# applied-geodesy/bundle-adjustment

Measured on AMD Instinct MI355X. Metric: LM iterations/sec, higher is better.
Workload: dtype f64

## Files before the change

bundle-adjustment_amd/csrc/cholflow.h:

```cpp
#pragma once
#include <hip/hip_runtime.h>
#include <limits.h>
#include <stddef.h>

#include <vector>

#include "devbuf.h"

namespace jaicov {

enum { FACTOR_DEFAULT = 0, FACTOR_STREAMS = 1, FACTOR_TWO_STEP = 2, FACTOR_ONE_KERNEL = 3, FACTOR_CHAIN2 = 4, FACTOR_CHAIN3 = 5 };

constexpr int HOOK_UNSET = INT_MIN;
struct FlowHooks {
    int form = FACTOR_DEFAULT;
    int min_blocks = HOOK_UNSET;
    int split_m = 0, split_from = 0;
    int timeout_ms = HOOK_UNSET;
    bool trace_on = false;
    int chain8_min_nb = HOOK_UNSET;
    bool chain_trace = false;
    bool verbose = false;
};
FlowHooks flow_hooks();

struct FlowDecision {
    bool use_flow;
    bool one_kernel;
    bool chain;
    int second;
    int split_m, split_from;
};
FlowDecision flow_decide(int nb, bool kernels_overlap, const FlowHooks &h);
int chain8_min_blocks(const FlowHooks &h);

enum { FLOW_TICKET = 0, FLOW_ABORT = 1, FLOW_DIAG_NEXT = 2, FLOW_CHAIN_AT = 3, FLOW_STALE = 4, FLOW_STALE_CONFIRMED = 5, FLOW_RESCUED = 6, FLOW_WG_OFF = 7, FLOW_CTRL_WORDS = 16 };
constexpr int FLOW_MAX_GRID = 1024;

struct FlowLayout {
    size_t done;
    size_t applied;
    size_t diag_ready;
    size_t factored;
    size_t wgstate;
    size_t wgsnap;
    size_t pflag;
    size_t words;
};
FlowLayout flow_layout(int nb, int row_blocks, int partials);

struct FlowView {
    double *L;
    long ld;
    double *invd;
    int *d_info;
    int nfact, n;
    hipStream_t stream;
    hipStream_t pstream;
    hipStream_t dstream;
};

struct FlowCounters { long long stale_events = 0, stale_confirmed = 0, rescued = 0; };

class FlowFactor {
  public:
    hipError_t init(const FlowView &view, const FlowHooks &hooks);
    bool ready() const { return ready_; }
    void set_source(const double *N, long ldN, const double *V, const double *Bh, int bstride, int d, int U) {
        src_ = N; src_ld_ = ldN; V_ = V; Bh_ = Bh; bstride_ = bstride; d_ = d; U_ = U;
    }
    hipError_t factor(hipEvent_t all_ready, bool profile);
    const int *abort_word() const { return ready_ ? flags_.get() + FLOW_ABORT : nullptr; }
    hipError_t read_ctrl(int (&cw)[8]) const;
    bool collect(const int (&cw)[8]);
    void report_stall() const;
    bool elapsed_ms(float *ms);
    hipError_t enable_trace(bool on);
    const long long *trace() const { return trace_.get(); }
    size_t trace_words() const { return ((size_t)n_tasks() + v_.nfact / 128) * 8; }
    int n_tasks() const { return (int)tasks_host_.size(); }
    const FlowCounters &counters() const { return counters_; }

  private:
    FlowView v_{};
    bool ready_ = false, timed_ = false;
    bool one_kernel_ = false, chain_ = false;
    int second_ = 0;
    int grid_ = 0;
    int keep_ = 0;
    int partials_ = 0;
    FlowLayout lay_{};
    int wg_off_ = 0;
    std::vector<int4> tasks_host_;
    DevBuf<int4> tasks_;
    DevBuf<int> flags_;
    DevBuf<double> scratch_;
    DevBuf<double> partial_;
    DevBuf<long long> trace_;
    DevBuf<double> diag_scratch_;
    HostMapped<int> alive_;
    int seq_ = 0;
    DevEvent e0_, e1_, t0_, t1_;
    const double *src_ = nullptr, *V_ = nullptr, *Bh_ = nullptr;
    long src_ld_ = 0;
    int d_ = 0, U_ = 0, bstride_ = 0;
    FlowCounters counters_;
};

}
```

bundle-adjustment_amd/csrc/cholflow.hip:

```cpp
#include <hip/hip_runtime.h>
#include <stdio.h>
#include <stdlib.h>
#include <string.h>

#include <algorithm>
#include <chrono>
#include <mutex>
#include <thread>
#include <vector>

#include "dense.h"
#include "gemm_f64.h"
#include "potrf_diag.h"

namespace jaicov {

#define HIPCHK(x)                                  \
    do {                                           \
        hipError_t _e = (x);                       \
        if (_e != hipSuccess) return _e;           \
    } while (0)

constexpr int FLOW_FIN = 1 << 20;
constexpr int FLOW_PART = 1 << 21;
// ... 3 lines not shown
constexpr int FLOW_STAGE = GEMM_BK * 2 * FLOW_LDS;

struct FlowArgs {
    double *L;
    long ld;
    double *invd;
    const int4 *tasks;
    int n_tasks;
    int nb;
    int fs;
    int *ctrl;
    int *done;
    int *applied;
    int *diag_ready;
    int *factored;
    int *info;
    int *alive;
    int seq;
    const double *src;
    long src_ld;
    const double *V;
    const double *Bh;
    int d, U, bstride;
    double *diag_scratch;
    const double *zeros;
    double *scratch;
    double *partial;
    int *pflag;
    long long timeout;
    int fake_a;
    int crit_prio;
    int keep;
    int second_wg;
    int second_update;
    int inv_wt;
    int crit_span;
    int *wgstate;
    long long *ctrace;
    long long *trace;
};

__device__ __forceinline__ int flow_ld(const int *p) { return __hip_atomic_load(p, __ATOMIC_RELAXED, __HIP_MEMORY_SCOPE_AGENT); }
__device__ __forceinline__ int flow_ld_rmw(const int *p) { return __hip_atomic_fetch_or(const_cast<int *>(p), 0, __ATOMIC_RELAXED, __HIP_MEMORY_SCOPE_AGENT); }
__device__ __forceinline__ void flow_st(int *p, int v) { __hip_atomic_store(p, v, __ATOMIC_RELAXED, __HIP_MEMORY_SCOPE_SYSTEM); }
__device__ __forceinline__ int flow_ld_sys(const int *p) { return __hip_atomic_load(p, __ATOMIC_RELAXED, __HIP_MEMORY_SCOPE_SYSTEM); }
__device__ __forceinline__ void store_wt(double *p, double v) {
// ... 191 lines not shown
                const double *src = phase != 0 || part ? g.zeros + (tq & 15)
                                    : scaled   ? g.src + ((long)ti * 128 + trow) * g.src_ld + (long)tj * 128 + tcol
                                               : g.L + ((long)ti * 128 + trow) * g.ld + (long)tj * 128 + tcol;
                const long sld = phase != 0 || part ? 0 : (scaled ? g.src_ld : g.ld);
#pragma unroll
                for (int x = 0; x < 4; x++)
#pragma unroll
                    for (int r = 0; r < 4; r++) {
                        const double *rowp = src + (long)(16 * x + 4 * r) * sld;
#pragma unroll
                        for (int y = 0; y < 4; y++) acc[x][y][r] = rowp[16 * y];
                    }
                if (scaled) {
                    const int R0 = ti * 128 + (int)trow, C0 = tj * 128 + (int)tcol;
                    double vc[4];
#pragma unroll
                    for (int y = 0; y < 4; y++) vc[y] = g.V[C0 + 16 * y];
#pragma unroll
                    for (int x = 0; x < 4; x++)
#pragma unroll
                        for (int r = 0; r < 4; r++) {
                            const int R = R0 + 16 * x + 4 * r;
                            const double vr = g.V[R];
#pragma unroll
                            for (int y = 0; y < 4; y++) {
                                const int Cc = C0 + 16 * y;
                                double v = vr * acc[x][y][r] * vc[y];
                                for (int a = 0; a < g.d; a++) v += g.Bh[(long)a * g.bstride + R] * g.Bh[(long)a * g.bstride + Cc];
                                const bool inside = R >= g.d && R < g.U && Cc >= g.d;
                                acc[x][y][r] = inside ? v : (R == Cc ? 1.0 : 0.0);
                            }
                        }
                }
            }
            if (g.trace && phase == 0) { t_c = wall_clock64(); c_c = clock64(); }
            for (bool more = true; more;) {
                const double *Ap, *Bp;
                long lda, ldb;
                int nk;
                double asign;
                if (phase == 0) {
                    if (k >= k1) break;
                    FLOW_STAGE_MARK(k, 3);
                    if (tid < 64) {
                        FLOW_OPAQUE_TID(lane);
                        const int *fi = g.done + (long)ti * g.fs, *fj = g.done + (long)tj * g.fs;
                        const long long t0 = wall_clock64();
                        int spins = 0, cnt = 0;
                        for (;;) {
                            const int idx = k + lane;
                            const bool ready = idx < k1 && flow_ld(fi + idx) != 0 && flow_ld(fj + idx) != 0;
                            const unsigned long long m = __ballot(ready);
                            cnt = m == ~0ull ? 64 : __builtin_ctzll(~m);
// ... 483 lines not shown
        if (tr) tr[4] = wall_clock64();
    }
}

FlowHooks flow_hooks() {
    FlowHooks h;
    if (const char *e = getenv("JAICOV_FACTOR_FORM")) {
        if (!strcmp(e, "streams")) h.form = FACTOR_STREAMS;
        else if (!strcmp(e, "two_step")) h.form = FACTOR_TWO_STEP;
        else if (!strcmp(e, "one_kernel")) h.form = FACTOR_ONE_KERNEL;
        else if (!strcmp(e, "chain2")) h.form = FACTOR_CHAIN2;
        else if (!strcmp(e, "chain3")) h.form = FACTOR_CHAIN3;
    }
    if (const char *e = getenv("JAICOV_FLOW_MIN_BLOCKS")) h.min_blocks = atoi(e);
    if (const char *e = getenv("JAICOV_FLOW_SPLIT")) {
        int a = 1, b = 0;
        if (sscanf(e, "%d:%d", &a, &b) >= 1) { h.split_m = a < 1 ? 1 : a; h.split_from = b; }
    }
    if (const char *e = getenv("JAICOV_FLOW_TIMEOUT_MS")) h.timeout_ms = atoi(e);
    h.trace_on = getenv("JAICOV_FLOW_TRACE_ON") != nullptr;
    if (const char *e = getenv("JAICOV_CHAIN8_MIN_NB")) h.chain8_min_nb = atoi(e);
    h.chain_trace = getenv("JAICOV_CHAIN_TRACE") != nullptr;
    h.verbose = getenv("JAICOV_VERBOSE") != nullptr;
    return h;
}

int chain8_min_blocks(const FlowHooks &h) { return h.chain8_min_nb != HOOK_UNSET ? h.chain8_min_nb : 24; }

FlowDecision flow_decide(int nb, bool kernels_overlap, const FlowHooks &h) {
    FlowDecision dec{};
    dec.use_flow = h.form != FACTOR_STREAMS && nb >= (h.min_blocks != HOOK_UNSET ? h.min_blocks : 12);
    if (dec.use_flow) {
        dec.one_kernel = !kernels_overlap || h.form == FACTOR_ONE_KERNEL;
        dec.chain = !dec.one_kernel && h.form != FACTOR_TWO_STEP;
        dec.second = dec.chain && h.form != FACTOR_CHAIN2 && (nb < 80 || h.form == FACTOR_CHAIN3) ? 2 : 0;
    }
    dec.split_m = 1; dec.split_from = 1 << 30;
    if (nb >= 80) { dec.split_m = 2; dec.split_from = nb / 2; }
    if (h.split_m > 0) { dec.split_m = h.split_m; dec.split_from = h.split_from; }
    return dec;
}

FlowLayout flow_layout(int nb, int row_blocks, int partials) {
    FlowLayout l{};
    l.done = FLOW_CTRL_WORDS;
    l.applied = l.done + (size_t)row_blocks * nb;
    l.diag_ready = l.applied + (size_t)row_blocks * nb;
    l.factored = l.diag_ready + nb;
    l.wgstate = l.factored + nb;
    l.wgsnap = l.wgstate + FLOW_MAX_GRID;
    l.pflag = l.wgsnap + FLOW_MAX_GRID;
    l.words = l.pflag + (size_t)partials;
    return l;
}

static std::vector<int4> flow_schedule(int nb, int row_blocks, int w, bool chain, int second, int split_m = 1, int split_from = 1 << 30, int *n_bufs = nullptr) {
    std::vector<int4> tasks;
    tasks.reserve((size_t)nb * (row_blocks + 1) / 2 + row_blocks);
    if (w < 1) w = 1;
    if (split_m > 8) split_m = 8;
    if (w > 1) split_m = 1;
    int bufs = 0;
    auto task = [&](int i, int j) {
// ... 34 lines not shown
    return tasks;
}

}
extern "C" int jaicov_debug_flow_tasks2(int nb, int row_blocks, int w, int chain, int second, int split_m, int split_from, int *out, int cap) {
    if (nb < 1 || row_blocks < nb) return -1;
    const std::vector<int4> t = jaicov::flow_schedule(nb, row_blocks, w, chain != 0, second, split_m, split_from);
    for (size_t q = 0; q < t.size() && (int)q < cap; q++) {
        out[4 * q] = t[q].x; out[4 * q + 1] = t[q].y; out[4 * q + 2] = t[q].z; out[4 * q + 3] = t[q].w;
    }
    return (int)t.size();
}
extern "C" int jaicov_debug_flow_tasks(int nb, int row_blocks, int w, int chain, int second, int *out, int cap) {
    return jaicov_debug_flow_tasks2(nb, row_blocks, w, chain, second, 1, 1 << 30, out, cap);
}
extern "C" void jaicov_debug_flow_split(int nb, int *m, int *from) {
    const jaicov::FlowDecision dec = jaicov::flow_decide(nb, true, jaicov::flow_hooks());
    *m = dec.split_m; *from = dec.split_from;
}
extern "C" void jaicov_debug_flow_decision(int nb, int kernels_overlap, int *out6) {
    const jaicov::FlowDecision dec = jaicov::flow_decide(nb, kernels_overlap != 0, jaicov::flow_hooks());
    out6[0] = dec.use_flow; out6[1] = dec.one_kernel; out6[2] = dec.chain; out6[3] = dec.second; out6[4] = dec.split_m; out6[5] = dec.split_from;
}
extern "C" int jaicov_debug_flow_layout(int nb, int row_blocks, int partials, long long *out8) {
    if (nb < 1 || row_blocks < nb || partials < 0) return -1;
    const jaicov::FlowLayout l = jaicov::flow_layout(nb, row_blocks, partials);
    const size_t w[8] = {l.done, l.applied, l.diag_ready, l.factored, l.wgstate, l.wgsnap, l.pflag, l.words};
    for (int i = 0; i < 8; i++) out8[i] = (long long)w[i];
    return jaicov::FLOW_MAX_GRID;
}
namespace jaicov {

__global__ void flow_probe_wait_kernel(int *word, int *result) {
    const long long t0 = wall_clock64();
    int seen = 0;
    while (wall_clock64() - t0 < 5000000LL) {
        if (__hip_atomic_load(word, __ATOMIC_RELAXED, __HIP_MEMORY_SCOPE_AGENT) != 0) { seen = 1; break; }
        __builtin_amdgcn_s_sleep(20);
    }
    *result = seen;
}
__global__ void flow_probe_set_kernel(int *word) { __hip_atomic_store(word, 1, __ATOMIC_RELAXED, __HIP_MEMORY_SCOPE_AGENT); }

static bool flow_kernels_overlap(hipStream_t dstream) {
    static int cached = -1;
    static std::mutex cache_mutex;
// ... 103 lines not shown
    return std::max(1, std::min(FLOW_MAX_GRID, 2 * (cus > 0 ? cus : 256)));
}
extern "C" int jaicov_debug_flow_residency(int *out8) {
    hipStream_t s = nullptr;
    StreamLease d(STREAM_DIAGONAL_CUS);
    if (!d.get() || hipStreamCreateWithFlags(&s, hipStreamNonBlocking) != hipSuccess) return -1;
    const FlowResidency r = flow_measure_residency(s, d.get(), flow_grid_size(), 2);
    hipStreamDestroy(s);
    out8[0] = r.valid; out8[1] = r.n_xcd; out8[2] = r.n_se; out8[3] = r.dealt; out8[4] = r.resident_min; out8[5] = r.queued_max; out8[6] = r.keep; out8[7] = r.se_cap;
    return 0;
}

hipError_t FlowFactor::init(const FlowView &view, const FlowHooks &hooks) {
    const int nb = view.nfact / 128, row_blocks = view.n / 128;
    if (!view.dstream) return hipErrorNotSupported;
    FlowFactor f;
    f.v_ = view;
    const bool overlap = hooks.form != FACTOR_ONE_KERNEL && flow_kernels_overlap(view.dstream);
    const FlowDecision dec = flow_decide(nb, overlap, hooks);
    f.one_kernel_ = dec.one_kernel; f.chain_ = dec.chain; f.second_ = dec.second;
    f.tasks_host_ = flow_schedule(nb, row_blocks, 1, f.chain_, f.second_, dec.split_m, dec.split_from, &f.partials_);
    HIPCHK(f.tasks_.reserve(f.tasks_host_.size()));
    HIPCHK(hipMemcpy(f.tasks_.get(), f.tasks_host_.data(), f.tasks_host_.size() * sizeof(int4), hipMemcpyHostToDevice));
    f.lay_ = flow_layout(nb, row_blocks, f.partials_);
    f.wg_off_ = (int)f.lay_.wgstate;
    if (f.flags_.reserve_finegrained(f.lay_.words) != hipSuccess) {
        (void)hipGetLastError();
        fprintf(stderr, "jaicov: no fine-grained device memory for the flags of the dataflow factorisation (%zu words): ordinary memory, rare stalls possible\n", f.lay_.words);
        HIPCHK(f.flags_.reserve(f.lay_.words));
    }
    HIPCHK(hipMemset(f.flags_.get(), 0, f.lay_.words * sizeof(int)));
    f.grid_ = flow_grid_size();
    HIPCHK(f.scratch_.reserve((size_t)f.grid_ * 16384 + 64));
    HIPCHK(hipMemset(f.scratch_.get() + (size_t)f.grid_ * 16384, 0, 64 * sizeof(double)));
    if (f.partials_ > 0) HIPCHK(f.partial_.reserve((size_t)f.partials_ * 16384));
    HIPCHK(f.alive_.alloc(4));
    for (int b = 0; b < 4; b++) f.alive_.get()[b] = 0;
    HIPCHK(f.e0_.create(hipEventDisableTiming));
    HIPCHK(f.e1_.create(hipEventDisableTiming));
    HIPCHK(f.t0_.create());
    HIPCHK(f.t1_.create());
    f.keep_ = f.chain_ ? flow_measure_residency(view.stream, view.dstream, f.grid_, f.second_ ? 3 : 2).keep : 0;
    f.ready_ = true;
    if (hooks.trace_on) HIPCHK(f.enable_trace(true));
    *this = std::move(f);
    return hipSuccess;
}

hipError_t FlowFactor::factor(hipEvent_t all_ready, bool profile) {
    const hipStream_t stream = v_.stream, dstream = v_.dstream;
    int *const flags = flags_.get();
    FlowArgs g{};
    g.L = v_.L; g.ld = v_.ld; g.invd = v_.invd;
    g.tasks = tasks_.get(); g.n_tasks = n_tasks(); g.nb = v_.nfact / 128; g.fs = g.nb;
    g.ctrl = flags;
    g.done = flags + lay_.done;
    g.applied = flags + lay_.applied;
    g.diag_ready = flags + lay_.diag_ready;
    g.factored = flags + lay_.factored;
    g.wgstate = flags + lay_.wgstate;
    g.pflag = flags + lay_.pflag;
    g.partial = partial_.get();
    g.info = v_.d_info;
    g.scratch = scratch_.get();
    g.zeros = scratch_.get() + (size_t)grid_ * 16384;
    const double expect_ms = (double)v_.nfact * v_.nfact * v_.nfact / 3.0 / 20e9;
    const FlowHooks now = flow_hooks();
    g.timeout = 100000LL * (now.timeout_ms != HOOK_UNSET ? now.timeout_ms : (int)(250 + 10 * expect_ms));
    g.src = src_; g.src_ld = src_ld_; g.V = V_; g.Bh = Bh_; g.d = d_; g.U = U_; g.bstride = bstride_;
    src_ = nullptr;
    g.trace = trace_.get();
    g.ctrace = trace_.get() ? trace_.get() + 8 * (size_t)n_tasks() : nullptr;
    g.fake_a = 0;
    g.crit_prio = 1;
    g.second_update = second_ >= 2 ? 1 : 0;
    g.second_wg = second_ ? 1 : 0;
    g.keep = chain_ ? keep_ : 0;
    g.inv_wt = 1;
    g.crit_span = chain_ ? 2 : 1;
    g.alive = alive_.get();
    g.seq = ++seq_;
    HIPCHK(hipMemsetAsync(flags, 0, lay_.words * sizeof(int), stream));
    HIPCHK(hipMemcpyAsync(flags + FLOW_WG_OFF, &wg_off_, sizeof(int), hipMemcpyHostToDevice, stream));
    HIPCHK(hipMemsetAsync(v_.d_info, 0, sizeof(int), stream));
    if (one_kernel_) {
        HIPCHK(diag_scratch_.reserve((size_t)grid_ * (128 * DP + 8 * 16 * WDP)));
        g.diag_scratch = diag_scratch_.get();
        g.alive = nullptr;
        if (all_ready) HIPCHK(hipStreamWaitEvent(stream, all_ready, 0));
        if (profile) HIPCHK(hipEventRecord(t0_.get(), stream));
        hipLaunchKernelGGL((chol_tile_kernel<1, true>), dim3(grid_), dim3(256), 0, stream, g);
        if (profile) {
            HIPCHK(hipEventRecord(t1_.get(), stream));
// ... 22 lines not shown
                    (void)hipStreamSynchronize(side);
                    (void)hipStreamSynchronize(dstream);
                    (void)hipEventRecord(e1_.get(), dstream);
                    (void)hipStreamWaitEvent(stream, e1_.get(), 0);
                    return hipErrorLaunchTimeOut;
                }
                if (waited_s > 2e-4) std::this_thread::yield();
            }
        }
    }
    if (profile) HIPCHK(hipEventRecord(t0_.get(), stream));
    hipLaunchKernelGGL((chol_tile_kernel<2, false>), dim3(grid_), dim3(256), 0, stream, g);
    if (profile) {
        HIPCHK(hipEventRecord(t1_.get(), stream));
        timed_ = true;
    }
    HIPCHK(hipEventRecord(e1_.get(), dstream));
    HIPCHK(hipStreamWaitEvent(stream, e1_.get(), 0));
    return hipGetLastError();
}

void FlowFactor::report_stall() const {
    if (!flags_.get()) return;
    const int nb = v_.nfact / 128, row_blocks = v_.n / 128;
    std::vector<int> f(lay_.words);
    if (hipMemcpy(f.data(), flags_.get(), lay_.words * sizeof(int), hipMemcpyDeviceToHost) != hipSuccess) return;
    const int *done = f.data() + lay_.done, *applied = f.data() + lay_.applied, *factored = f.data() + lay_.factored;
    int c_inv = 0, c_fac = 0, c_sub = 0;
    while (c_inv < nb && done[(size_t)c_inv * nb + c_inv]) ++c_inv;
    while (c_fac < nb && factored[c_fac]) ++c_fac;
    while (c_sub + 1 < nb && done[(size_t)(c_sub + 1) * nb + c_sub]) ++c_sub;
    int first_open = -1, open_row = -1;
    for (int j = 0; j < nb && first_open < 0; j++)
        for (int i = j + 1; i < row_blocks; i++)
            if (!done[(size_t)i * nb + j]) { first_open = j; open_row = i; break; }
    fprintf(stderr,
            "jaicov: dataflow factorisation abandoned (abort %d): ticket %d of %d, chain form %d, blocks %d; inverses published %d, "
            "factors published %d, subdiagonal tiles published %d, first unfinished tile (%d, %d), chain workgroup at column %d stage %d",
            f[FLOW_ABORT], f[FLOW_TICKET], n_tasks(), (int)chain_, nb, c_inv, c_fac, c_sub, open_row, first_open, f[FLOW_CHAIN_AT] >> 4, f[FLOW_CHAIN_AT] & 15);
    if (chain_ && c_fac < nb) {
        const int c = c_fac > 0 ? c_fac - 1 : 0;
        if (c + 1 < nb)
            fprintf(stderr, "; column %d: tile below stored with %d updates, next diagonal tile with %d (wanted %d)", c,
                    applied[(size_t)(c + 1) * nb + c] - 1, applied[(size_t)(c + 1) * nb + c + 1] - 1, c);
    }
    fprintf(stderr, "\n");
    for (int b = 0; b < 3; b++) {
        const unsigned hw = (unsigned)f[8 + 2 * b];
        if (chain_ && (b < 2 || second_))
            fprintf(stderr, "jaicov:   chain workgroup %d runs on [xcc %d se %u sh %u cu %u]\n", b, f[9 + 2 * b] - 1, (hw >> 13) & 7, (hw >> 12) & 1, (hw >> 8) & 0xf);
    }
    const int *wg = f.data() + lay_.wgstate, *snap = f.data() + lay_.wgsnap;
    std::vector<std::pair<int, int>> open;
    for (int b = 0; b < grid_; b++)
        if (wg[b] != 0 && (wg[b] & 15) != 7) open.push_back({wg[b] >> 12, b});
    std::sort(open.begin(), open.end());
    std::vector<long long> tr;
    if (trace_.get()) {
        tr.resize((size_t)n_tasks() * 8);
        if (hipMemcpy(tr.data(), trace_.get(), tr.size() * sizeof(long long), hipMemcpyDeviceToHost) != hipSuccess) tr.clear();
    }
    long long t_last = 0;
    for (size_t q = 0; q + 7 < tr.size(); q += 8) t_last = std::max(t_last, tr[q + 3]);
    auto ticket_of = [&](int i, int j) {
        for (int t = 0; t < n_tasks(); t++)
            if (tasks_host_[t].x == i && tasks_host_[t].y == j) return t;
        return -1;
    };
    {
        int by_stage[16] = {0};
        std::vector<std::pair<int, int>> busy;
        for (int b = 0; b < grid_; b++) {
            const int w = snap[b];
            if (w == 0) continue;
            by_stage[w & 15]++;
            if ((w & 15) == 4 || (w & 15) == 5 || (w & 15) == 6 || (w & 15) == 1) busy.push_back({w >> 12, b});
        }
        std::sort(busy.begin(), busy.end());
        fprintf(stderr, "jaicov:   when the first wait ran out: workgroups by stage [1 drawn %d, 2 waits for a visit / the inverse %d, 3 polls operands %d, 4 products %d, 5 / 6 stores %d / %d, 7 between tasks %d, 9 waits for partial sums %d]\n",
                by_stage[1], by_stage[2], by_stage[3], by_stage[4], by_stage[5], by_stage[6], by_stage[7], by_stage[9]);
        for (size_t q = 0; q < busy.size() && q < 8; q++) {
            const int w = snap[busy[q].second], t = w >> 12;
            const int4 tk = (t >= 0 && t < (int)tasks_host_.size()) ? tasks_host_[t] : make_int4(-1, -1, 0, 0);
            fprintf(stderr, "jaicov:     not waiting then: workgroup %d, ticket %d = tile (%d, %d)%s, stage %d at block column %d; now: stage %d at block column %d\n", busy[q].second, t, tk.x, tk.y,
                    (tk.w & FLOW_PART) ? " partial sum" : "", w & 15, (w >> 4) & 255, wg[busy[q].second] & 15, (wg[busy[q].second] >> 4) & 255);
        }
    }
    for (size_t q = 0; q < open.size() && q < 6; q++) {
        const int w = wg[open[q].second], t = w >> 12;
        const int4 tk = tasks_host_.empty() ? make_int4(-1, -1, 0, 0) : tasks_host_[t];
        fprintf(stderr, "jaicov:   workgroup %d: ticket %d = tile (%d, %d) to block column %d%s, stage %d at block column %d\n", open[q].second, t, tk.x,
                tk.y, tk.w & (FLOW_FIN - 1), (tk.w & FLOW_FIN) ? " + finish" : "", w & 15, (w >> 4) & 255);
        const int kk = (w >> 4) & 255;
        if (!tr.empty() && (w & 15) == 8 && kk < tk.y)
            for (int side = 0; side < 2; side++) {
                const int oi = side == 0 ? tk.x : tk.y, ot = ticket_of(oi, kk);
                if (ot < 0) continue;
                const long long *r = &tr[(size_t)ot * 8];
                const unsigned hw = (unsigned)(r[7] & 0xffffffff);
                const int ws = snap[(int)(r[6] & 0xffff)];
                fprintf(stderr, "jaicov:     (when the first wait ran out that workgroup was at: ticket %d, block column %d, stage %d)\n", ws >> 12, (ws >> 4) & 255, ws & 15);
                fprintf(stderr, "jaicov:     operand tile (%d, %d) = ticket %d on workgroup %d [xcc %d se %u sh %u cu %u simd %u wave %u]: started %.3f ms, tile loaded %.3f ms, updates done %.3f ms, finished %.3f ms before the end; it waited %.3f ms\n",
                        oi, kk, ot, (int)(r[6] & 0xffff), (int)((r[7] >> 32) & 0xf), (hw >> 13) & 7, (hw >> 12) & 1, (hw >> 8) & 0xf, (hw >> 4) & 3, hw & 0xf,
                        (t_last - r[0]) / 1e5, (t_last - r[1]) / 1e5, (t_last - r[2]) / 1e5, r[3] ? (t_last - r[3]) / 1e5 : -1.0, r[4] / 1e5);
            }
    }
}

hipError_t FlowFactor::enable_trace(bool on) {
    if (on && !trace_.get()) {
        HIPCHK(trace_.reserve(trace_words()));
        HIPCHK(hipMemset(trace_.get(), 0, trace_words() * sizeof(long long)));
    } else if (!on) {
// ... 24 lines not shown
```

bundle-adjustment_amd/csrc/dense.h:

```cpp
#pragma once
#include <hip/hip_runtime.h>
#include <stdint.h>

#include <map>
#include <vector>

#include "cholflow.h"
#include "devbuf.h"

namespace jaicov {

struct GemmArgs;

constexpr int DENSE_NB = 128;
constexpr int DENSE_MAX_RHS = 8;
constexpr int DENSE_PANEL = 512;

enum { STREAM_PLAIN = 0, STREAM_HIGH_PRIORITY = 1, STREAM_UPDATE_CUS = 2, STREAM_DIAGONAL_CUS = 3, STREAM_KINDS = 4 };
constexpr int STREAM_MASKED_IDLE_MAX = 2;
hipStream_t stream_acquire(int kind);
void stream_release(int kind, hipStream_t s);
int device_cu_count();
class StreamLease {
    int kind_ = STREAM_PLAIN;
// ... 41 lines not shown
    struct Store { DevBuf<double> L, invd, pm, xch, W, Q; DevBuf<int> info; } store;
    FlowHooks hooks;
    bool profile = false;
    std::vector<DevEvent> prof_ev;
    std::vector<double> prof_flops;
    size_t prof_used = 0;
    double stat_launches = 0, stat_ms = 0, stat_flops = 0;
    void prof_collect();
    double flops_order = 0;

    FlowFactor flow;
    hipError_t potrf_streams(hipEvent_t first_ready, hipEvent_t all_ready);

    hipError_t init(hipStream_t s, int n_padded, bool with_inverse, bool with_rhs_rows = false, const DenseSolver *share = nullptr);
    hipError_t acquire(bool with_inverse, const DenseSolver *share);
    ~DenseSolver() { release(); }
    double *rhs_row(int q) const { return L + (long)(nfact + q) * ld; }
    void release();
    hipError_t panel(hipStream_t st, int K0, int K1);
    hipError_t timed_gemm(hipStream_t st, const GemmArgs &u, double flops, int small = 0);
    hipError_t potrf(hipEvent_t first_ready = nullptr, hipEvent_t all_ready = nullptr);
    hipError_t begin_refactor();
    int first_panel_cols() const;
    hipError_t backsolve_aug(double *X, long xs, int nrhs);
    hipError_t solve_rhs(const double *b, double *tmp, double *X);
    hipError_t trtri();
    hipError_t lauum();
    hipError_t symmetrize(double *M);
    int fetch_info();
};

}
```

bundle-adjustment_amd/csrc/dense.hip:

```cpp
#include "dense.h"

#include <math.h>
#include <stdio.h>
#include <stdlib.h>
#include <string.h>

#include <algorithm>
#include <map>
#include <mutex>
#include <vector>

#include "gemm_f64.h"
#include "potrf_diag.h"

namespace jaicov {

#define HIPCHK(x)                                  \
    do {                                           \
        hipError_t _e = (x);                       \
        if (_e != hipSuccess) return _e;           \
    } while (0)

__global__ __launch_bounds__(256) void potrf_diag_kernel(double *A, long ld, double *inv_out, int *info, int blk, int dbg) {
    __shared__ double S[128 * DP];
// ... 1045 lines not shown
        p.M = p.N = p.K = 128; p.alpha = 1.0; p.beta = 0.0; p.kmode = KMODE_FULL;
        p.batch_sum_limit = nb - 1;
        HIPCHK(gemm_f64(stream, LAY_KC, LAY_XC, p, nb - 1, 0, 0, std::min(CH_PM, nb - 1)));
        GemmArgs f{};
        f.A = L + (long)128 * ld; f.lda = ld; f.strideA = 128 * (ld + 1); f.strideA2 = (long)128 * ld;
        f.B = invd + 16384; f.ldb = 128; f.strideB = 16384; f.strideB2 = 16384;
        f.C = pm + (size_t)CH_PM * nb * 16384 + 16384; f.ldc = 128; f.strideC = 16384; f.strideC2 = (long)nb * 16384 + 16384;
        f.M = f.N = f.K = 128; f.alpha = 1.0; f.beta = 0.0; f.kmode = KMODE_FULL;
        f.batch_sum_limit = nb - 1;
        if (pstream && pm_e0.get() && pm_done.get()) {
            HIPCHK(hipEventRecord(pm_e0.get(), stream));
            HIPCHK(hipStreamWaitEvent(pstream, pm_e0.get(), 0));
            HIPCHK(gemm_f64(pstream, LAY_XC, LAY_KC, f, nb - 1, 0, 0, std::min(CH_PM, nb - 1)));
            HIPCHK(hipEventRecord(pm_done.get(), pstream));
            pm_wait = true;
        } else {
            HIPCHK(gemm_f64(stream, LAY_XC, LAY_KC, f, nb - 1, 0, 0, std::min(CH_PM, nb - 1)));
        }
    }
    pm_ready = true;
    return hipGetLastError();
}

hipError_t DenseSolver::backsolve_aug(double *X, long xs, int nrhs) {
    if (!aug || nrhs < 1 || nrhs > DENSE_MAX_RHS) return hipErrorInvalidValue;
    const int nb = nfact / 128;
    HIPCHK(hipMemsetAsync(X, 0xFF, (size_t)nrhs * xs * sizeof(double), stream));
    const int *ab = flow.abort_word();
    if (nrhs <= 1 && pm && nb >= chain8_min_blocks(flow_hooks())) {
        HIPCHK(premultiply());
        HIPCHK(launch_chain8(rhs_row(0), X, ab, nullptr));
    } else if (nrhs <= 1) hipLaunchKernelGGL(backsolve_chain_kernel<1>, dim3(nb), dim3(256), 0, stream, L, ld, invd, rhs_row(0), ld, X, xs, nb, nrhs, ab);
    else if (nrhs <= 2) hipLaunchKernelGGL(backsolve_chain_kernel<2>, dim3(nb), dim3(256), 0, stream, L, ld, invd, rhs_row(0), ld, X, xs, nb, nrhs, ab);
    else if (nrhs <= 4) hipLaunchKernelGGL(backsolve_chain_kernel<4>, dim3(nb), dim3(256), 0, stream, L, ld, invd, rhs_row(0), ld, X, xs, nb, nrhs, ab);
    else hipLaunchKernelGGL(backsolve_chain_kernel<8>, dim3(nb), dim3(256), 0, stream, L, ld, invd, rhs_row(0), ld, X, xs, nb, nrhs, ab);
    return hipGetLastError();
}

hipError_t DenseSolver::solve_rhs(const double *b, double *tmp, double *X) {
    const int nb = nfact / 128;
    HIPCHK(hipMemsetAsync(tmp, 0xFF, (size_t)nfact * sizeof(double), stream));
    HIPCHK(hipMemsetAsync(X, 0xFF, (size_t)nfact * sizeof(double), stream));
    if (pm && nb >= chain8_min_blocks(flow_hooks())) {
        HIPCHK(premultiply());
        const bool tracing = hooks.chain_trace;
        DevBuf<long long> trbuf;
// ... 220 lines not shown
```

bundle-adjustment_amd/csrc/engine.hip:

```cpp
#include <hip/hip_runtime.h>
#include <math.h>
#include <stdio.h>
#include <string.h>

#include <algorithm>
#include <atomic>
#include <chrono>
#include <string>
#include <vector>

#include "../../include/jaicov_dense.h"
#include "../../include/jaicov_neq.h"
#include "ba_kernels.h"
#include "batchinv.h"
#include "create_plan.h"
#include "datum.h"
#include "dense.h"
#include "devbuf.h"
#include "gemm_f64.h"
#include "reliability.h"
#include "transform.h"

namespace jaicov {
hipError_t launch_rows(hipStream_t, const DevProblem &, const double *, int, int, double *, double *);
// ... 203 lines not shown
    double *d_V = nullptr, *d_B = nullptr, *d_dx = nullptr;
    double *d_cc_partial = nullptr;
    double *d_omega = nullptr, *d_G = nullptr, *d_H = nullptr, *d_F = nullptr, *d_E = nullptr;
    int32_t *d_idx = nullptr;
    DenseSolver solver;
    bool solver_has_inverse = false;
    enum { ST_NEW, ST_PARAMS, ST_ACCUMULATED, ST_BUILT, ST_SOLVED } state = ST_NEW;
    bool have_Q = false, rows_valid = false, reduced = false;
    bool deterministic = true;
    std::atomic<int> cancel{0};
    bool sim_built = false;
    double lambda_used = 0.0;
    std::vector<double> hB;
    double timings[8] = {0, 0, 0, 0, 0, 0, 0, 0};
    double create_ms[8] = {0, 0, 0, 0, 0, 0, 0, 0};
    hipEvent_t ev[10] = {};
    bool pp_plain_ok = false;
    hipEvent_t ev_first = nullptr, ev_all = nullptr;
    hipEvent_t ev_r0 = nullptr, ev_r1 = nullptr;
    jaicov::XformState *xform = nullptr;
    jaicov::RelState *rel = nullptr;
    const double *d_ll_diag = nullptr;
    double sigma2_acc = 0.0;
    double q_sigma2 = 0.0, q_lambda = 0.0;
    std::vector<double> q_vals;
    jaicov::DatumState *datum = nullptr;
};

#define FAIL(e, code, msg)                 \
    do {                                   \
        (e)->err = (msg);                  \
        return (code);                     \
    } while (0)
#define HIPE(e, x)                                                                        \
    do {                                                                                  \
        hipError_t _err = (x);                                                            \
        if (_err != hipSuccess) {                                                         \
            (e)->err = std::string(#x) + ": " + hipGetErrorString(_err);                  \
            return _err == hipErrorOutOfMemory ? JAICOV_ERR_OUT_OF_MEMORY : JAICOV_ERR_DEVICE; \
        }                                                                                 \
    } while (0)
#define TRY(x) do { const int _rc = (x); if (_rc) return _rc; } while (0)

template <typename T, typename P>
static int upload(jaicov_engine *e, const T *src, size_t count, P **dst) {
    *dst = nullptr;
// ... 806 lines not shown
    }
    int apply_correction(const RefineBorder &bd, const std::vector<double> &dl, double *dx_out) {
        float ms1 = 0.f;
        hipEventElapsedTime(&ms1, e->ev_r0, e->ev_r1);
        refine_ms += ms1;
        double dk[7] = {0, 0, 0, 0, 0, 0, 0};
        border_multipliers(dl.data(), bd.rk, dk);
        double cmax = 0.0, xmax = 0.0;
        for (int c = d; c < U; c++) {
            double dy = dl[c];
            for (int a = 0; a < d; a++) dy -= X[(size_t)(1 + a) * vs + c] * dk[a];
            const double corr = e->h_V[c] * dy;
            if (!std::isfinite(corr)) FAIL(e, JAICOV_ERR_NOT_FINITE, "non-finite refinement step");
            dx_out[c] += corr;
            cmax = std::max(cmax, fabs(corr)); xmax = std::max(xmax, fabs(dx_out[c]));
        }
        for (int a = 0; a < d; a++) dx_out[a] += R[a] * dk[a];
        e->last_refine_correction = xmax > 0.0 ? cmax / xmax : 0.0;
        return JAICOV_OK;
    }
    int factor_and_substitute() {
        const int nrhs = d + 1;
        const bool fused = slv.flow.ready();
        const int c1 = std::min(slv.first_panel_cols(), Up);
        int info = 0;
        for (int attempt = 0;; attempt++) {
            HIPE(e, slv.begin_refactor());
            if (!fused)
                hipLaunchKernelGGL(scale_copy_kernel, dim3((c1 + 255) / 256, Up), dim3(256), 0, e->stream, e->d_N, (long)Upad, slv.L, ld, U,
                                   Up, d, e->d_V, e->d_B, Upad, 0, c1);
            HIPE(e, hipMemsetAsync(slv.rhs_row(0), 0, (size_t)128 * ld * sizeof(double), e->stream));
            hipLaunchKernelGGL(scale_vec_kernel, dim3((Up + 255) / 256), dim3(256), 0, e->stream, e->d_n, e->d_V, slv.rhs_row(0), U, Up, d);
            if (d > 0)
                HIPE(e, hipMemcpy2DAsync(slv.rhs_row(1), (size_t)ld * sizeof(double), e->d_B, (size_t)Upad * sizeof(double),
                                         (size_t)Up * sizeof(double), (size_t)d, hipMemcpyDeviceToDevice, e->stream));
            HIPE(e, hipEventRecord(e->ev_first, e->stream));
            if (!fused && c1 < Up)
                hipLaunchKernelGGL(scale_copy_kernel, dim3((Up - c1 + 255) / 256, Up), dim3(256), 0, e->stream, e->d_N, (long)Upad, slv.L,
                                   ld, U, Up, d, e->d_V, e->d_B, Upad, c1, Up);
            HIPE(e, hipEventRecord(e->ev_all, e->stream));
            if (fused) slv.flow.set_source(e->d_N, (long)Upad, e->d_V, e->d_B, Upad, d, U);
            HIPE(e, slv.potrf(e->ev_first, e->ev_all));
            HIPE(e, hipEventRecord(e->ev[5], e->stream));
            HIPE(e, slv.backsolve_aug(e->d_G, vs, nrhs));
            HIPE(e, hipEventRecord(e->ev[6], e->stream));
            X.assign((size_t)nrhs * vs, 0.0);
            HIPE(e, hipMemcpyAsync(X.data(), e->d_G, X.size() * sizeof(double), hipMemcpyDeviceToHost, e->stream));
            fast_refined = false;
            if (d == 0 && e->refine_steps >= 1 && !e->sim_built) {
                TRY(refine_begin());
                hipLaunchKernelGGL(scale_vec_kernel, dim3((Up + 255) / 256), dim3(256), 0, e->stream, e->d_G, e->d_V, e->d_dx, U, Up, 0);
                TRY(refine_step(RefineBorder{}, delta0));
                fast_refined = true;
            }
            info = slv.fetch_info();
            if (info == -9 && attempt < 2) {
                ++e->flow_retries;
                fprintf(stderr, "jaicov: factorisation abandoned on the device (a wait ran into its time limit); repeating it (%d)\n", attempt + 1);
                continue;
            }
            break;
        }
        if (info < 0) FAIL(e, JAICOV_ERR_DEVICE, "factorisation did not complete on the device (code " + std::to_string(info) + ")");
        if (info != 0) FAIL(e, JAICOV_ERR_SINGULAR, "normal-equation matrix is singular / not positive definite at pivot " + std::to_string(info));
        return JAICOV_OK;
    }
// ... 424 lines not shown
extern "C" int jaicov_neq_set_profiling(jaicov_engine *e, int enable) {
    if (!e) return JAICOV_ERR_BAD_ARGUMENT;
    e->solver.profile = enable != 0;
    return JAICOV_OK;
}

extern "C" int jaicov_neq_kernel_stats(jaicov_engine *e, double *stats, int32_t n, int reset) {
    if (!e || !stats || n < 3) return JAICOV_ERR_BAD_ARGUMENT;
    stats[0] = e->solver.stat_launches; stats[1] = e->solver.stat_ms; stats[2] = e->solver.stat_flops;
    if (n >= 6) { stats[3] = e->dm_stat_passes; stats[4] = e->dm_stat_ms; stats[5] = e->dm_stat_flops; }
    if (n >= 10) {
        stats[6] = (double)e->flow_retries;
        const FlowCounters &c = e->solver.flow.counters(), &cS = e->solverS.flow.counters();
        stats[7] = (double)(c.stale_events + cS.stale_events);
        stats[8] = (double)(c.stale_confirmed + cS.stale_confirmed);
        stats[9] = (double)(c.rescued + cS.rescued);
    }
    if (n >= 11) stats[10] = e->last_refine_correction;
    if (n >= 12) stats[11] = (double)e->refine_steps;
    if (n >= 13) stats[12] = (double)e->pp.cw;
    if (reset) e->solver.stat_launches = e->solver.stat_ms = e->solver.stat_flops = e->dm_stat_passes = e->dm_stat_ms = e->dm_stat_flops = 0.0;
    return JAICOV_OK;
}

extern "C" int jaicov_neq_create_timings(jaicov_engine *e, double *ms, int32_t n) {
    if (!e || !ms) return JAICOV_ERR_BAD_ARGUMENT;
    for (int i = 0; i < n && i < 8; i++) ms[i] = e->create_ms[i];
    return JAICOV_OK;
}

extern "C" int jaicov_neq_get_block_weight(jaicov_engine *e, int32_t block, double *out, size_t len) {
    if (!e || !out) return JAICOV_ERR_BAD_ARGUMENT;
    if (!e->h_caller_block.empty()) {
        int internal = -1;
        for (size_t g = 0; g < e->h_caller_block.size(); g++)
            if (e->h_caller_block[g] == block) internal = (int)g;
        block = internal;
    }
    if (block < 0 || block >= (int)e->h_blk_mine.size() || !e->h_blk_mine[block]) FAIL(e, JAICOV_ERR_BAD_ARGUMENT, "no such image block on this engine");
    const int b = e->h_blk_ip_begin[block], mpts = e->h_blk_ip_begin[block + 1] - b, m = 2 * mpts;
    if (len != (size_t)m * m) FAIL(e, JAICOV_ERR_BAD_ARGUMENT, "len must be (2 * points of the block)^2");
    HIPE(e, hipSetDevice(e->device));
    if (e->h_blk_w_off[block] < 0) FAIL(e, JAICOV_ERR_BAD_ARGUMENT, "this block has no dispersion of its own");
    std::vector<double> w((size_t)m * m);
    HIPE(e, hipMemcpy(w.data(), e->p.blk_w + e->h_blk_w_off[block], w.size() * sizeof(double), hipMemcpyDeviceToHost));
    const int32_t *perm = e->h_perm_local.empty() ? nullptr : e->h_perm_local.data() + b;
// ... 345 lines not shown
```

Measured before the change: 38.65.

## Place right-hand sides in the factor's padding rows instead of an extra block row

When the padded gap between U and the factor size can hold the right-hand sides, the fused source loader writes the scaled normal vector and border columns into the padding rows, with a huge pivot on their diagonal. The factorisation then runs the smaller task schedule with no extra block row, and a small kernel copies the forward-substituted rows out before the back-substitution. This removes the memset, scale and 2D copy of the separate RHS block row and the extra row-block tile updates. The cost is reliance on the large-pivot trick staying numerically clean and a second task list.

```diff
diff --git a/bundle-adjustment_amd/csrc/cholflow.h b/bundle-adjustment_amd/csrc/cholflow.h
--- a/bundle-adjustment_amd/csrc/cholflow.h
+++ b/bundle-adjustment_amd/csrc/cholflow.h
@@ -21,6 +21,7 @@
     int chain8_min_nb = HOOK_UNSET;
     bool chain_trace = false;
     bool verbose = false;
+    bool rhs_block_row = false;
 };
 FlowHooks flow_hooks();
 
@@ -33,6 +34,9 @@
 };
 FlowDecision flow_decide(int nb, bool kernels_overlap, const FlowHooks &h);
 int chain8_min_blocks(const FlowHooks &h);
+
+bool flow_rhs_in_padding(int U, int nfact, int nrhs, int invert, const FlowHooks &h);
+constexpr double FLOW_RHS_PIVOT = 0x1p200;
 
 enum { FLOW_TICKET = 0, FLOW_ABORT = 1, FLOW_DIAG_NEXT = 2, FLOW_CHAIN_AT = 3, FLOW_STALE = 4, FLOW_STALE_CONFIRMED = 5, FLOW_RESCUED = 6, FLOW_WG_OFF = 7, FLOW_CTRL_WORDS = 16 };
 constexpr int FLOW_MAX_GRID = 1024;
@@ -66,9 +70,13 @@
   public:
     hipError_t init(const FlowView &view, const FlowHooks &hooks);
     bool ready() const { return ready_; }
-    void set_source(const double *N, long ldN, const double *V, const double *Bh, int bstride, int d, int U) {
-        src_ = N; src_ld_ = ldN; V_ = V; Bh_ = Bh; bstride_ = bstride; d_ = d; U_ = U;
+    void set_source(const double *N, long ldN, const double *V, const double *Bh, int bstride, int d, int U, const double *rhs_n = nullptr) {
+        src_ = N; src_ld_ = ldN; V_ = V; Bh_ = Bh; bstride_ = bstride; d_ = d; U_ = U; rhs_n_ = rhs_n;
     }
+    bool rhs_in_padding(int U, int nrhs, int invert) const {
+        return ready_ && !one_kernel_ && !tasks_pad_host_.empty() && flow_rhs_in_padding(U, v_.nfact, nrhs, invert, flow_hooks());
+    }
+    bool last_in_padding() const { return last_pad_; }
     hipError_t factor(hipEvent_t all_ready, bool profile);
     const int *abort_word() const { return ready_ ? flags_.get() + FLOW_ABORT : nullptr; }
     hipError_t read_ctrl(int (&cw)[8]) const;
@@ -93,6 +101,9 @@
     int wg_off_ = 0;
     std::vector<int4> tasks_host_;
     DevBuf<int4> tasks_;
+    std::vector<int4> tasks_pad_host_;
+    DevBuf<int4> tasks_pad_;
+    bool last_pad_ = false;
     DevBuf<int> flags_;
     DevBuf<double> scratch_;
     DevBuf<double> partial_;
@@ -101,7 +112,7 @@
     HostMapped<int> alive_;
     int seq_ = 0;
     DevEvent e0_, e1_, t0_, t1_;
-    const double *src_ = nullptr, *V_ = nullptr, *Bh_ = nullptr;
+    const double *src_ = nullptr, *V_ = nullptr, *Bh_ = nullptr, *rhs_n_ = nullptr;
     long src_ld_ = 0;
     int d_ = 0, U_ = 0, bstride_ = 0;
     FlowCounters counters_;
diff --git a/bundle-adjustment_amd/csrc/cholflow.hip b/bundle-adjustment_amd/csrc/cholflow.hip
--- a/bundle-adjustment_amd/csrc/cholflow.hip
+++ b/bundle-adjustment_amd/csrc/cholflow.hip
@@ -49,6 +49,7 @@
     const double *V;
     const double *Bh;
     int d, U, bstride;
+    const double *rhs_n;
     double *diag_scratch;
     const double *zeros;
     double *scratch;
@@ -286,13 +287,20 @@
                         for (int r = 0; r < 4; r++) {
                             const int R = R0 + 16 * x + 4 * r;
                             const double vr = g.V[R];
+                            const int q = R - g.U;
+                            const bool rhs = g.rhs_n != nullptr && q >= 0 && q <= g.d;
 #pragma unroll
                             for (int y = 0; y < 4; y++) {
                                 const int Cc = C0 + 16 * y;
                                 double v = vr * acc[x][y][r] * vc[y];
                                 for (int a = 0; a < g.d; a++) v += g.Bh[(long)a * g.bstride + R] * g.Bh[(long)a * g.bstride + Cc];
                                 const bool inside = R >= g.d && R < g.U && Cc >= g.d;
-                                acc[x][y][r] = inside ? v : (R == Cc ? 1.0 : 0.0);
+                                v = inside ? v : (R == Cc ? 1.0 : 0.0);
+                                if (rhs)
+                                    v = Cc >= g.U ? (R == Cc ? FLOW_RHS_PIVOT : 0.0)
+                                        : q > 0   ? g.Bh[(long)(q - 1) * g.bstride + Cc]
+                                                  : (Cc >= g.d ? vc[y] * g.rhs_n[Cc] : 0.0);
+                                acc[x][y][r] = v;
                             }
                         }
                 }
@@ -822,6 +830,7 @@
     if (const char *e = getenv("JAICOV_CHAIN8_MIN_NB")) h.chain8_min_nb = atoi(e);
     h.chain_trace = getenv("JAICOV_CHAIN_TRACE") != nullptr;
     h.verbose = getenv("JAICOV_VERBOSE") != nullptr;
+    if (const char *e = getenv("JAICOV_RHS_FORM")) h.rhs_block_row = !strcmp(e, "block_row");
     return h;
 }
 
@@ -839,6 +848,10 @@
     if (nb >= 80) { dec.split_m = 2; dec.split_from = nb / 2; }
     if (h.split_m > 0) { dec.split_m = h.split_m; dec.split_from = h.split_from; }
     return dec;
+}
+
+bool flow_rhs_in_padding(int U, int nfact, int nrhs, int invert, const FlowHooks &h) {
+    return !h.rhs_block_row && invert == 0 && nrhs >= 1 && nrhs <= 8 && U > 0 && nfact - U >= nrhs && nfact - U < 128;
 }
 
 FlowLayout flow_layout(int nb, int row_blocks, int partials) {
@@ -919,6 +932,9 @@
     const jaicov::FlowDecision dec = jaicov::flow_decide(nb, kernels_overlap != 0, jaicov::flow_hooks());
     out6[0] = dec.use_flow; out6[1] = dec.one_kernel; out6[2] = dec.chain; out6[3] = dec.second; out6[4] = dec.split_m; out6[5] = dec.split_from;
 }
+extern "C" int jaicov_debug_rhs_in_padding(int U, int nfact, int nrhs, int invert) {
+    return jaicov::flow_rhs_in_padding(U, nfact, nrhs, invert, jaicov::flow_hooks()) ? 1 : 0;
+}
 extern "C" int jaicov_debug_flow_layout(int nb, int row_blocks, int partials, long long *out8) {
     if (nb < 1 || row_blocks < nb || partials < 0) return -1;
     const jaicov::FlowLayout l = jaicov::flow_layout(nb, row_blocks, partials);
@@ -1068,6 +1084,11 @@
     f.tasks_host_ = flow_schedule(nb, row_blocks, 1, f.chain_, f.second_, dec.split_m, dec.split_from, &f.partials_);
     HIPCHK(f.tasks_.reserve(f.tasks_host_.size()));
     HIPCHK(hipMemcpy(f.tasks_.get(), f.tasks_host_.data(), f.tasks_host_.size() * sizeof(int4), hipMemcpyHostToDevice));
+    if (row_blocks > nb) {
+        f.tasks_pad_host_ = flow_schedule(nb, nb, 1, f.chain_, f.second_, dec.split_m, dec.split_from);
+        HIPCHK(f.tasks_pad_.reserve(f.tasks_pad_host_.size()));
+        HIPCHK(hipMemcpy(f.tasks_pad_.get(), f.tasks_pad_host_.data(), f.tasks_pad_host_.size() * sizeof(int4), hipMemcpyHostToDevice));
+    }
     f.lay_ = flow_layout(nb, row_blocks, f.partials_);
     f.wg_off_ = (int)f.lay_.wgstate;
     if (f.flags_.reserve_finegrained(f.lay_.words) != hipSuccess) {
@@ -1098,7 +1119,9 @@
     int *const flags = flags_.get();
     FlowArgs g{};
     g.L = v_.L; g.ld = v_.ld; g.invd = v_.invd;
-    g.tasks = tasks_.get(); g.n_tasks = n_tasks(); g.nb = v_.nfact / 128; g.fs = g.nb;
+    last_pad_ = src_ != nullptr && rhs_n_ != nullptr && !one_kernel_ && !tasks_pad_host_.empty();
+    g.tasks = last_pad_ ? tasks_pad_.get() : tasks_.get(); g.n_tasks = (int)(last_pad_ ? tasks_pad_host_ : tasks_host_).size();
+    g.nb = v_.nfact / 128; g.fs = g.nb;
     g.ctrl = flags;
     g.done = flags + lay_.done;
     g.applied = flags + lay_.applied;
@@ -1114,7 +1137,8 @@
     const FlowHooks now = flow_hooks();
     g.timeout = 100000LL * (now.timeout_ms != HOOK_UNSET ? now.timeout_ms : (int)(250 + 10 * expect_ms));
     g.src = src_; g.src_ld = src_ld_; g.V = V_; g.Bh = Bh_; g.d = d_; g.U = U_; g.bstride = bstride_;
-    src_ = nullptr;
+    g.rhs_n = last_pad_ ? rhs_n_ : nullptr;
+    src_ = nullptr; rhs_n_ = nullptr;
     g.trace = trace_.get();
     g.ctrace = trace_.get() ? trace_.get() + 8 * (size_t)n_tasks() : nullptr;
     g.fake_a = 0;
@@ -1183,7 +1207,8 @@
 
 void FlowFactor::report_stall() const {
     if (!flags_.get()) return;
-    const int nb = v_.nfact / 128, row_blocks = v_.n / 128;
+    const int nb = v_.nfact / 128, row_blocks = last_pad_ ? nb : v_.n / 128;
+    const std::vector<int4> &list = last_pad_ ? tasks_pad_host_ : tasks_host_;
     std::vector<int> f(lay_.words);
     if (hipMemcpy(f.data(), flags_.get(), lay_.words * sizeof(int), hipMemcpyDeviceToHost) != hipSuccess) return;
     const int *done = f.data() + lay_.done, *applied = f.data() + lay_.applied, *factored = f.data() + lay_.factored;
@@ -1198,7 +1223,7 @@
     fprintf(stderr,
             "jaicov: dataflow factorisation abandoned (abort %d): ticket %d of %d, chain form %d, blocks %d; inverses published %d, "
             "factors published %d, subdiagonal tiles published %d, first unfinished tile (%d, %d), chain workgroup at column %d stage %d",
-            f[FLOW_ABORT], f[FLOW_TICKET], n_tasks(), (int)chain_, nb, c_inv, c_fac, c_sub, open_row, first_open, f[FLOW_CHAIN_AT] >> 4, f[FLOW_CHAIN_AT] & 15);
+            f[FLOW_ABORT], f[FLOW_TICKET], (int)list.size(), (int)chain_, nb, c_inv, c_fac, c_sub, open_row, first_open, f[FLOW_CHAIN_AT] >> 4, f[FLOW_CHAIN_AT] & 15);
     if (chain_ && c_fac < nb) {
         const int c = c_fac > 0 ? c_fac - 1 : 0;
         if (c + 1 < nb)
@@ -1224,8 +1249,8 @@
     long long t_last = 0;
     for (size_t q = 0; q + 7 < tr.size(); q += 8) t_last = std::max(t_last, tr[q + 3]);
     auto ticket_of = [&](int i, int j) {
-        for (int t = 0; t < n_tasks(); t++)
-            if (tasks_host_[t].x == i && tasks_host_[t].y == j) return t;
+        for (int t = 0; t < (int)list.size(); t++)
+            if (list[t].x == i && list[t].y == j) return t;
         return -1;
     };
     {
@@ -1242,14 +1267,14 @@
                 by_stage[1], by_stage[2], by_stage[3], by_stage[4], by_stage[5], by_stage[6], by_stage[7], by_stage[9]);
         for (size_t q = 0; q < busy.size() && q < 8; q++) {
             const int w = snap[busy[q].second], t = w >> 12;
-            const int4 tk = (t >= 0 && t < (int)tasks_host_.size()) ? tasks_host_[t] : make_int4(-1, -1, 0, 0);
+            const int4 tk = (t >= 0 && t < (int)list.size()) ? list[t] : make_int4(-1, -1, 0, 0);
             fprintf(stderr, "jaicov:     not waiting then: workgroup %d, ticket %d = tile (%d, %d)%s, stage %d at block column %d; now: stage %d at block column %d\n", busy[q].second, t, tk.x, tk.y,
                     (tk.w & FLOW_PART) ? " partial sum" : "", w & 15, (w >> 4) & 255, wg[busy[q].second] & 15, (wg[busy[q].second] >> 4) & 255);
         }
     }
     for (size_t q = 0; q < open.size() && q < 6; q++) {
         const int w = wg[open[q].second], t = w >> 12;
-        const int4 tk = tasks_host_.empty() ? make_int4(-1, -1, 0, 0) : tasks_host_[t];
+        const int4 tk = list.empty() ? make_int4(-1, -1, 0, 0) : list[t];
         fprintf(stderr, "jaicov:   workgroup %d: ticket %d = tile (%d, %d) to block column %d%s, stage %d at block column %d\n", open[q].second, t, tk.x,
                 tk.y, tk.w & (FLOW_FIN - 1), (tk.w & FLOW_FIN) ? " + finish" : "", w & 15, (w >> 4) & 255);
         const int kk = (w >> 4) & 255;
diff --git a/bundle-adjustment_amd/csrc/dense.h b/bundle-adjustment_amd/csrc/dense.h
--- a/bundle-adjustment_amd/csrc/dense.h
+++ b/bundle-adjustment_amd/csrc/dense.h
@@ -87,6 +87,7 @@
     hipError_t potrf(hipEvent_t first_ready = nullptr, hipEvent_t all_ready = nullptr);
     hipError_t begin_refactor();
     int first_panel_cols() const;
+    hipError_t take_rhs_from_padding(int U, int nrhs);
     hipError_t backsolve_aug(double *X, long xs, int nrhs);
     hipError_t solve_rhs(const double *b, double *tmp, double *X);
     hipError_t trtri();
diff --git a/bundle-adjustment_amd/csrc/dense.hip b/bundle-adjustment_amd/csrc/dense.hip
--- a/bundle-adjustment_amd/csrc/dense.hip
+++ b/bundle-adjustment_amd/csrc/dense.hip
@@ -1091,6 +1091,17 @@
     return hipGetLastError();
 }
 
+__global__ void rhs_from_padding_kernel(const double *__restrict__ L, long ld, double *__restrict__ Z, int U, int nfact) {
+    const int c = blockIdx.x * blockDim.x + threadIdx.x;
+    if (c >= nfact) return;
+    Z[(long)blockIdx.y * ld + c] = c < U ? L[(long)(U + blockIdx.y) * ld + c] : 0.0;
+}
+hipError_t DenseSolver::take_rhs_from_padding(int U, int nrhs) {
+    if (!aug || nrhs < 1 || nrhs > DENSE_MAX_RHS || U < 1 || U + nrhs > nfact) return hipErrorInvalidValue;
+    hipLaunchKernelGGL(rhs_from_padding_kernel, dim3((nfact + 255) / 256, nrhs), dim3(256), 0, stream, L, ld, rhs_row(0), U, nfact);
+    return hipGetLastError();
+}
+
 hipError_t DenseSolver::backsolve_aug(double *X, long xs, int nrhs) {
     if (!aug || nrhs < 1 || nrhs > DENSE_MAX_RHS) return hipErrorInvalidValue;
     const int nb = nfact / 128;
diff --git a/bundle-adjustment_amd/csrc/engine.hip b/bundle-adjustment_amd/csrc/engine.hip
--- a/bundle-adjustment_amd/csrc/engine.hip
+++ b/bundle-adjustment_amd/csrc/engine.hip
@@ -249,6 +249,7 @@
     jaicov::RelState *rel = nullptr;
     const double *d_ll_diag = nullptr;
     double sigma2_acc = 0.0;
+    bool rhs_in_padding = false;
     double q_sigma2 = 0.0, q_lambda = 0.0;
     std::vector<double> q_vals;
     jaicov::DatumState *datum = nullptr;
@@ -1101,6 +1102,8 @@
     int factor_and_substitute() {
         const int nrhs = d + 1;
         const bool fused = slv.flow.ready();
+        const bool in_padding = fused && slv.flow.rhs_in_padding(U, nrhs, invert);
+        e->rhs_in_padding = in_padding;
         const int c1 = std::min(slv.first_panel_cols(), Up);
         int info = 0;
         for (int attempt = 0;; attempt++) {
@@ -1108,19 +1111,22 @@
             if (!fused)
                 hipLaunchKernelGGL(scale_copy_kernel, dim3((c1 + 255) / 256, Up), dim3(256), 0, e->stream, e->d_N, (long)Upad, slv.L, ld, U,
                                    Up, d, e->d_V, e->d_B, Upad, 0, c1);
-            HIPE(e, hipMemsetAsync(slv.rhs_row(0), 0, (size_t)128 * ld * sizeof(double), e->stream));
-            hipLaunchKernelGGL(scale_vec_kernel, dim3((Up + 255) / 256), dim3(256), 0, e->stream, e->d_n, e->d_V, slv.rhs_row(0), U, Up, d);
-            if (d > 0)
-                HIPE(e, hipMemcpy2DAsync(slv.rhs_row(1), (size_t)ld * sizeof(double), e->d_B, (size_t)Upad * sizeof(double),
-                                         (size_t)Up * sizeof(double), (size_t)d, hipMemcpyDeviceToDevice, e->stream));
+            if (!in_padding) {
+                HIPE(e, hipMemsetAsync(slv.rhs_row(0), 0, (size_t)128 * ld * sizeof(double), e->stream));
+                hipLaunchKernelGGL(scale_vec_kernel, dim3((Up + 255) / 256), dim3(256), 0, e->stream, e->d_n, e->d_V, slv.rhs_row(0), U, Up, d);
+                if (d > 0)
+                    HIPE(e, hipMemcpy2DAsync(slv.rhs_row(1), (size_t)ld * sizeof(double), e->d_B, (size_t)Upad * sizeof(double),
+                                             (size_t)Up * sizeof(double), (size_t)d, hipMemcpyDeviceToDevice, e->stream));
+            }
             HIPE(e, hipEventRecord(e->ev_first, e->stream));
             if (!fused && c1 < Up)
                 hipLaunchKernelGGL(scale_copy_kernel, dim3((Up - c1 + 255) / 256, Up), dim3(256), 0, e->stream, e->d_N, (long)Upad, slv.L,
                                    ld, U, Up, d, e->d_V, e->d_B, Upad, c1, Up);
             HIPE(e, hipEventRecord(e->ev_all, e->stream));
-            if (fused) slv.flow.set_source(e->d_N, (long)Upad, e->d_V, e->d_B, Upad, d, U);
+            if (fused) slv.flow.set_source(e->d_N, (long)Upad, e->d_V, e->d_B, Upad, d, U, in_padding ? e->d_n : nullptr);
             HIPE(e, slv.potrf(e->ev_first, e->ev_all));
             HIPE(e, hipEventRecord(e->ev[5], e->stream));
+            if (in_padding) HIPE(e, slv.take_rhs_from_padding(U, nrhs));
             HIPE(e, slv.backsolve_aug(e->d_G, vs, nrhs));
             HIPE(e, hipEventRecord(e->ev[6], e->stream));
             X.assign((size_t)nrhs * vs, 0.0);
@@ -1591,6 +1597,8 @@
     if (reset) e->solver.stat_launches = e->solver.stat_ms = e->solver.stat_flops = e->dm_stat_passes = e->dm_stat_ms = e->dm_stat_flops = 0.0;
     return JAICOV_OK;
 }
+
+extern "C" int jaicov_debug_rhs_form(jaicov_engine *e) { return e ? (e->rhs_in_padding ? 1 : 0) : -1; }
 
 extern "C" int jaicov_neq_create_timings(jaicov_engine *e, double *ms, int32_t n) {
     if (!e || !ms) return JAICOV_ERR_BAD_ARGUMENT;
```

Result: slower. 38.16 (-1.3%).
